# bcgsc/goldrush

Measured on AMD Instinct MI355X. Metric: reads/s through GoldRush-Path (hash + miBF query), higher is better.
Workload: dtype u64

## Files before the change

### goldrush_amd/csrc/grp_device.h

```cpp
#pragma once
#include <hip/hip_runtime.h>
#include <stdint.h>

#define GRP_DEV_MAX_H 16
#define GRP_DEV_MAX_W 32
#define GRP_BUCKET_IDS 13u
#define GRP_NEAR_CW 8u
#define GRP_UNIT_U4 8u
#define GRP_UNIT_DW 32u
#define GRP_UNIT_QW 16u
#define GRP_SUPER_SHIFT 22
#define GRP_CHUNK_BUCKETS 4096u

struct DevSeeds
{
  uint32_t h;
  uint32_t k;
  uint32_t wmax;
  uint32_t n_left;
  uint32_t wide;
  uint32_t weight[GRP_DEV_MAX_H];
  uint32_t span[GRP_DEV_MAX_H];
  uint32_t shift[GRP_DEV_MAX_H][GRP_DEV_MAX_W];
  ulonglong2 tab[GRP_DEV_MAX_H][GRP_DEV_MAX_W][4];
};

struct DevFilter
{
  uint32_t* bv;
  uint4* buckets;
  const uint64_t* super;
  ulonglong2* far;
  uint64_t far_mask;
  unsigned long long* ovf_keys;
  uint32_t* ovf_ids;
  uint64_t ovf_mask;
  uint64_t m;
  uint64_t m_inv;
  uint64_t w_magic;
  uint64_t n_buckets;
  uint64_t pop;
  uint32_t W;
  uint32_t pad;
};

constexpr unsigned long long GRP_CNT_MASK = (1ull << 28) - 1ull;
constexpr uint32_t GRP_EPOCH_MAX = (1u << 10) - 1u;

__host__ __device__ inline uint32_t
grp_cnt(unsigned long long w)
{
  return (uint32_t)(w & GRP_CNT_MASK);
}

__host__ __device__ inline unsigned long long
grp_cnt_with(unsigned long long w, uint32_t count)
{
#if defined(__HIP_DEVICE_COMPILE__)
// ... 163 lines not shown
```

### goldrush_amd/csrc/grp_kernels.inc

```

__device__ inline uint64_t
window_lo(const uint32_t* sBases, uint32_t b)
{
  uint32_t bit = b * 2u;
  uint32_t wi = bit >> 5;
  uint32_t sh = bit & 31u;
  uint64_t lo = (uint64_t)sBases[wi] | ((uint64_t)sBases[wi + 1] << 32);
  uint64_t w = lo >> sh;
  if (sh) {
    w |= (uint64_t)sBases[wi + 2] << (64u - sh);
  }
  return w;
}

struct Win
{
  uint64_t lo;
  const uint32_t* src;
  uint32_t b;
};

__device__ inline Win
window_at(const uint32_t* sBases, uint32_t b)
{
// ... 532 lines not shown
    slot = (slot + 1u) & mask;
  }
}

__device__ inline void
hist_add16(uint32_t* keys, uint32_t* cnt_words, uint32_t cap, uint32_t id, uint32_t* sDistinct, uint32_t limit, uint32_t* sOverflow)
{
  if (*reinterpret_cast<volatile uint32_t*>(sDistinct) >= limit) {
    *sOverflow = 1u;
    return;
  }
  uint32_t slot = __umulhi(id * 2654435761u, cap);
  for (;;) {
    uint32_t old = atomicCAS(&keys[slot], 0u, id);
    if (old == 0u) {
      atomicAdd(sDistinct, 1u);
    }
    if (old == 0u || old == id) {
      atomicAdd(&cnt_words[slot >> 1], 1u << ((slot & 1u) << 4));
      return;
    }
    slot = (slot + 1u == cap) ? 0u : slot + 1u;
  }
}

__device__ inline bool
better(uint32_t c, uint32_t id, uint32_t bc, uint32_t bid)
{
  return (c > bc) || (c == bc && c != 0u && id < bid);
}

template<int WT, bool LEFT, bool RIGHT>
__device__ inline void
seed_halves(const ulonglong2* sTab, const DevSeeds* __restrict__ sd, uint32_t n_left, const Win& win, uint64_t& L, uint64_t& RL, uint64_t& R, uint64_t& RR)
{
  const uint64_t w = win.lo;
  L = RL = R = RR = 0;
  const uint32_t wt = WT > 0 ? (uint32_t)WT : sd->weight[0];
  if (n_left == 8u && wt == 16u) {
    if constexpr (LEFT) {
#pragma unroll
      for (uint32_t i = 0; i < 8u; ++i) {
        const ulonglong2 e = sTab[i * 4u + ((uint32_t)(w >> sd->shift[0][i]) & 3u)];
        L ^= e.x;
        RL ^= e.y;
      }
    }
    if constexpr (RIGHT) {
#pragma unroll
      for (uint32_t i = 8u; i < 16u; ++i) {
        const ulonglong2 e = sTab[i * 4u + ((uint32_t)(w >> sd->shift[0][i]) & 3u)];
        R ^= e.x;
        RR ^= e.y;
      }
    }
    return;
  }
  if constexpr (LEFT) {
    for (uint32_t i = 0; i < n_left; ++i) {
      const ulonglong2 e = sTab[i * 4u + ((uint32_t)(w >> sd->shift[0][i]) & 3u)];
      L ^= e.x;
      RL ^= e.y;
    }
  }
  if constexpr (RIGHT) {
    for (uint32_t i = n_left; i < wt; ++i) {
      const ulonglong2 e = sTab[i * 4u + ((uint32_t)(w >> sd->shift[0][i]) & 3u)];
      R ^= e.x;
      RR ^= e.y;
    }
  }
}

__device__ inline uint64_t
srol_small(uint64_t x, uint32_t n)
{
  const uint64_t M33 = 0x1FFFFFFFFULL, M31 = 0x7FFFFFFFULL;
  const uint64_t lo = x & M33, hi = x >> 33;
  return ((((hi << n) | (hi >> (31u - n))) & M31) << 33) | (((lo << n) | (lo >> (33u - n))) & M33);
}

#define GRP_TILE_FLAGGED 0xFFFFFFFFu

__device__ inline void
store_coherent(unsigned long long* p, unsigned long long v)
{
  __hip_atomic_store(p, v, __ATOMIC_RELAXED, __HIP_MEMORY_SCOPE_AGENT);
}

__device__ inline unsigned long long
load_coherent(const unsigned long long* p)
{
  return __hip_atomic_load(p, __ATOMIC_RELAXED, __HIP_MEMORY_SCOPE_AGENT);
}

__device__ inline uint32_t
ldc(const uint32_t* p)
{
  return __hip_atomic_load(p, __ATOMIC_RELAXED, __HIP_MEMORY_SCOPE_AGENT);
}

__device__ inline void
// ... 1316 lines not shown
  return best_old;
}

template<int H, int FR, int WT, bool ST, bool VER = false, bool GT = false>
__global__ void __launch_bounds__(THREADS, (ST && H <= 3) ? 3 : ((!ST && H >= 4 && H <= 5) ? 3 : 1))
k_query(DevFilter f,
        DevReads rd,
        const DevSeeds* __restrict__ sd,
        uint32_t tile_len,
        uint64_t tile_begin,
        const uint32_t* __restrict__ tile_idx,
        uint32_t hist_cap,
        uint32_t distinct_limit,
        grp_tile_summary* __restrict__ tiles_out,
        grp_id_count* __restrict__ lists_out,
        uint64_t lists_cap,
        unsigned long long* __restrict__ ctr,
        uint32_t* __restrict__ flagged_out,
        uint32_t flagged_cap,
        uint32_t direct_stride,
        uint32_t blk0,
        DevStreamCtl sc,
        DevBatchView bv,
        uint32_t* __restrict__ gtab = nullptr)
{
  if constexpr (VER && !ST) {
    if (bv.redo_count != nullptr && blockIdx.x >= *bv.redo_count) {
      return;
    }
  }
  extern __shared__ uint4 smem4[];
  ulonglong2* sTab = reinterpret_cast<ulonglong2*>(smem4);
  const uint32_t hn = frame_seeds<H>(sd);
  uint32_t* sKeys;
  uint32_t* sCnts;
  uint32_t* sBases;
  if constexpr (GT) {
    sKeys = gtab + (size_t)blockIdx.x * (hist_cap + hist_cap / 2u);
    sCnts = sKeys + hist_cap;
    sBases = reinterpret_cast<uint32_t*>(sTab + hn * sd->wmax * 4u);
  } else {
    sKeys = reinterpret_cast<uint32_t*>(sTab + hn * sd->wmax * 4u);
    sCnts = sKeys + hist_cap;
    sBases = sCnts + hist_cap / 2u;
  }
  auto tab_word = [&](const uint32_t* p) -> uint32_t {
    if constexpr (GT) {
      return __hip_atomic_load(p, __ATOMIC_RELAXED, __HIP_MEMORY_SCOPE_AGENT);
    } else {
      return *p;
    }
  };
  __shared__ uint32_t sListN, sDistinct, sOverflow, sListOff, sListW;
  __shared__ uint32_t sRed[2 * (THREADS / 64)];
  __shared__ uint32_t sBest[2 * (THREADS / 64)];
  __shared__ uint32_t sTile;
  __shared__ unsigned long long sDirectWord;
  __shared__ uint32_t sInsWave[THREADS / 64 + 1];
  __shared__ uint32_t sEv, sAct;
  __shared__ uint32_t sHeldTile[2], sHeldPasses[2];
  __shared__ uint32_t sBuf;
  __shared__ uint32_t sCut;
  __shared__ uint32_t sOwnRedo[2], sOwnRedoN;
  __shared__ uint32_t sWalkEnd;
  __shared__ uint32_t sGen;

  load_tab(sTab, sd);
  constexpr uint32_t STREAM_STOP = 0x40000000u;
  uint32_t nxt = 0;
  uint32_t stop = 0;
  uint32_t my_ev = 0;
  uint32_t phase = 0;
  bool host_abort_seen = false;
  uint32_t ev_next = 0;
  uint32_t pending_event = 0;
  uint32_t* const sFp = (ST && sc.ctl && sc.n_fp) ? reinterpret_cast<uint32_t*>(reinterpret_cast<char*>(smem4) + sc.fp_off) : nullptr;
  if constexpr (ST) {
    if (threadIdx.x == 0) {
      sHeldTile[0] = sHeldTile[1] = STREAM_REDO_NONE;
      sHeldPasses[0] = sHeldPasses[1] = 0u;
      sBuf = 0u;
      sCut = 0u;
      sOwnRedoN = 0u;
      sWalkEnd = 0u;
      sGen = 1u;
      if (sc.dbg) {
        stc(&sc.dbg[blockIdx.x], 0x00000001u);
        stc(&sc.dbg[4095], gridDim.x);
        stc(&sc.dbg[4096 + (blockIdx.x & 1023u)], (uint32_t)wall_clock64());
        stc(&sc.dbg[5120 + (blockIdx.x & 1023u)], (__builtin_amdgcn_s_getreg((16 - 1) << 11 | 4) & 0xFFFFu) | (__builtin_amdgcn_s_getreg((4 - 1) << 11 | 20) << 16));
      }
      if (__hip_atomic_load(sc.abort_host, __ATOMIC_RELAXED, __HIP_MEMORY_SCOPE_SYSTEM)) {
        atomicMin(sc.park, 0u);
        atomicMax(sc.next_tile, STREAM_STOP);
        __hip_atomic_store(sc.abort, 1u, __ATOMIC_RELAXED, __HIP_MEMORY_SCOPE_AGENT);
        stop = 1u;
        host_abort_seen = true;
      }
      if (sc.ctl) {
        uint32_t ph0 = 0;
// ... 220 lines not shown

  uint32_t n_hit = 0, n_miss = 0;
  uint32_t last[H];
#pragma unroll
  for (int s = 0; s < H; ++s) {
    last[s] = Lp - sd->span[s];
  }
  const uint32_t sub = threadIdx.x & 3u;
  const uint32_t quad_base = (threadIdx.x & 63u) & ~3u;

  const uint32_t n_left = (H >= 2 && H <= GRP_H_GROUP && WT != GRP_WT_LONG) ? sd->n_left : 0u;
  constexpr uint32_t OV = (uint32_t)H - 1u, USE = 64u - OV;
  static_assert(THREADS == 256, "the helper-lane layout below is written for four waves per workgroup (my_wave == 3 is the last one, FBH = 3 * USE + 64)");
  constexpr uint32_t FBH = 3u * USE + 64u;
  const uint32_t ftile = frames_per_tile(sd, tile_len);
  const bool helper = n_left != 0u && (ftile + FBH * FR - 1u) / (FBH * FR) == (ftile + THREADS * FR - 1u) / (THREADS * FR);
  const uint32_t FB = helper ? FBH : (uint32_t)THREADS;
  const uint32_t my_wave = threadIdx.x >> 6, my_lane = threadIdx.x & 63u;
  const uint32_t my_off = helper ? (my_wave * USE + my_lane) : threadIdx.x;
  const bool my_real = helper ? (my_wave == 3u || my_lane < USE) : true;
  const bool my_tail_wave = helper ? my_wave == 3u : true;
  const uint32_t passes = (frames + FB * FR - 1u) / (FB * FR);
  uint64_t bk[FR][H];
  uint32_t off[FR][H];
  bool live_j[FR];
  auto positions = [&](uint32_t pp, uint64_t (&bk_)[FR][H], uint32_t (&off_)[FR][H], bool (&lv)[FR]) {
  if (n_left != 0u) {
#pragma unroll
    for (int j = 0; j < FR; ++j) {
      const uint32_t fr_raw = (pp * FR + j) * FB + my_off;
      const uint32_t fr = min(fr_raw, frames - 1u);
      lv[j] = my_real && fr_raw < frames;
      uint64_t hL, hRL, hR, hRR;
      seed_halves<WT, true, true>(sTab, sd, n_left, window_at(sBases, boff + fr), hL, hRL, hR, hRR);
      const uint64_t hv0 = (hL ^ hR) + (hRL ^ hRR);
#pragma unroll
      for (int s = 0; s < H; ++s) {
        uint64_t hv = hv0;
        if (s != 0) {
          uint64_t nR = __shfl_down((unsigned long long)hR, (unsigned)s, 64);
          uint64_t nRR = __shfl_down((unsigned long long)hRR, (unsigned)s, 64);
          if (my_tail_wave && my_lane + (uint32_t)s >= 64u) {
            uint64_t a, b;
            seed_halves<WT, false, true>(sTab, sd, n_left, window_at(sBases, boff + min(fr_raw + (uint32_t)s, frames - 1u)), a, b, nR, nRR);
          }
          if (lv[j]) {
            if (fr <= last[s]) {
              hv = (srol_small(hL, (uint32_t)s) ^ nR) + (hRL ^ srol_small(nRR, (uint32_t)s));
            } else {
              hv = seed_hash_t<WT>(sTab, sd, s, window_at(sBases, boff + last[s]));
            }
          }
        }
        const Probe p = grp_locate(f, hv);
        bk_[j][s] = p.b;
        off_[j][s] = p.off;
        if constexpr (ST) {
          if (fp_cur != nullptr) {
            fp_cur[((pp * FR + (uint32_t)j) * (uint32_t)THREADS + threadIdx.x) * (uint32_t)H + (uint32_t)s] = lv[j] ? slot_fp(p.b, p.off) : 0u;
          }
        }
      }
    }
  } else {
#pragma unroll
    for (int j = 0; j < FR; ++j) {
      const uint32_t fr_raw = (pp * FR + j) * THREADS + threadIdx.x;
      const uint32_t fr = min(fr_raw, frames - 1u);
      lv[j] = fr_raw < frames;
#pragma unroll
      for (int s = 0; s < H; ++s) {
        if (!seed_on<H>(s, frame_seeds<H>(sd))) {
          bk_[j][s] = 0;
          off_[j][s] = 0;
          if constexpr (ST) {
            if (fp_cur != nullptr) {
              fp_cur[((pp * FR + (uint32_t)j) * (uint32_t)THREADS + threadIdx.x) * (uint32_t)H + (uint32_t)s] = 0u;
            }
// ... 794 lines not shown
```

### goldrush_amd/csrc/grpath_hip.hip

```cpp
#include "grp_device.h"
#include "host/gr_tiles_core.hpp"

#include "../../include/grpath.h"

#include <algorithm>
#include <cstdarg>
#include <cstdio>
#include <cstring>
#include <functional>
#include <chrono>
#include <cmath>
#include <mutex>
#include <string>
#include <thread>
#include <vector>


namespace {

thread_local std::string g_create_error;

struct EventPair
{
  hipEvent_t a, b;
  int kind;
};

}


struct QuerySlot
{
  grp_tile_summary* d_tiles = nullptr;
  uint64_t d_tiles_cap = 0;
// ... 375 lines not shown
      c->kstat[ep.kind].ms += (double)ms;
    }
    c->free_events.push_back(ep);
  }
  c->pending.swap(keep);
}

uint64_t
next_pow2_64(uint64_t v)
{
  uint64_t p = 1;
  while (p < v) {
    p <<= 1;
  }
  return p;
}

uint32_t
next_pow2(uint64_t v)
{
  uint32_t p = 1;
  while (p < v) {
    p <<= 1;
  }
  return p;
}

size_t
tab_bytes(const grp_ctx* c)
{
  return (size_t)c->h_seeds.h * c->h_seeds.wmax * 4u * sizeof(ulonglong2);
}

constexpr size_t
bases_bytes(uint32_t nbases)
{
  size_t words = (nbases + 15u) / 16u + 1u + 4u;
  return ((words * 4u + 15u) / 16u) * 16u;
}

inline bool
long_span(const grp_ctx* c)
{
  return c->h_seeds.wide > 1u;
}

inline uint32_t
span0(const grp_ctx* c)
{
  return c->h_seeds.span[0];
}

inline uint32_t
tile_frames(const grp_ctx* c)
{
  return c->params.tile + c->params.k - span0(c);
}

inline uint32_t
tile_parts(const grp_ctx* c)
{
  return (tile_frames(c) + THREADS - 1) / THREADS;
}

template<typename K>
int
// ... 56 lines not shown
  sl.h_qctr = nullptr;
  sl.dec_cap = 0;
  HIP_TRY(c, hipMalloc(&sl.d_dec_raw, (cap + 2) * sizeof(grp_read_decision)));
  HIP_TRY(c, hipHostMalloc(&sl.h_dec_raw, (cap + 2) * sizeof(grp_read_decision), hipHostMallocDefault));
  memset(sl.h_dec_raw, 0, 2 * sizeof(grp_read_decision));
  sl.d_dec = sl.d_dec_raw + 2;
  sl.h_dec = sl.h_dec_raw + 2;
  sl.h_qctr = reinterpret_cast<uint64_t*>(sl.h_dec_raw);
  sl.dec_cap = cap;
  return GRP_OK;
}

template<typename T>
int ensure_dev(grp_ctx* c, T*& p, uint64_t& cap, uint64_t want);

constexpr size_t LDS_PER_WORKGROUP = 160 * 1024 - 512;
static_assert(GRP_DEV_MAX_H * GRP_DEV_MAX_W * 4u * sizeof(ulonglong2) + bases_bytes(GRP_MAX_TILE + GRP_MAX_SPAN + GRP_DEV_MAX_H) <= LDS_PER_WORKGROUP,
              "a tile of the longest span does not fit the LDS beside the seed tables");
constexpr uint32_t GT_SLICE = 256;

struct QueryGeom
{
  uint32_t hist_cap;
  uint32_t distinct_limit;
  size_t lds;
  bool global_table = false;
};

QueryGeom
query_geom(const grp_ctx* c, bool full)
{
  const uint32_t h = c->params.h, tile = c->params.tile;
  const uint64_t max_ids = (uint64_t)tile_frames(c) * h;
  auto lds_of = [&](uint32_t cap) { return tab_bytes(c) + (size_t)cap * 6 + bases_bytes(tile + c->params.k + h); };
  const uint32_t cap_full = (uint32_t)((max_ids + (uint64_t)THREADS * h + 2 + 1023) / 1024 * 1024);
  const uint32_t forced_small = c->env_small_hist;
  QueryGeom g;
  g.hist_cap = cap_full;
  if (!full) {
    if (forced_small && forced_small < cap_full && forced_small > (uint32_t)THREADS * h + 64) {
      g.hist_cap = forced_small;
    } else if (lds_of(cap_full) > 52 * 1024) {
      const size_t fixed = lds_of(0);
      const uint32_t cap = (uint32_t)((52 * 1024 - std::min<size_t>(fixed, 40 * 1024)) / 6 / 1024 * 1024);
      if (cap > (uint32_t)THREADS * h + 1024 && cap < cap_full) {
        g.hist_cap = cap;
      }
    }
    if (g.hist_cap == cap_full && lds_of(cap_full) > LDS_PER_WORKGROUP) {
      const size_t fixed = lds_of(0);
      const uint32_t cap = fixed < LDS_PER_WORKGROUP ? (uint32_t)((LDS_PER_WORKGROUP - fixed) / 6 / 1024 * 1024) : 0u;
      if (cap > (uint32_t)THREADS * h + 64) {
        g.hist_cap = cap;
      }
    }
  }
  g.distinct_limit = g.hist_cap - THREADS * h - 1;
  g.lds = lds_of(g.hist_cap);
  if (full && g.lds > LDS_PER_WORKGROUP) {
    g.global_table = true;
    g.lds = lds_of(0);
  }
  return g;
}

template<int HH, int QWT>
int
launch_query_wt(grp_ctx* c, const grp_reads* r, uint64_t n_launch, uint64_t t0, const uint32_t* d_tile_idx, const QueryGeom& g, uint64_t list_cap, grp_tile_summary* out_tiles, grp_id_count* out_lists, uint32_t direct_stride, const DevStreamCtl* stream_ctl,
                uint32_t blk0, bool list_flags, bool plain)
{
  if (!out_tiles) {
    out_tiles = c->q->d_tiles;
    out_lists = c->q->d_lists;
  }
  size_t launch_lds = g.lds;
  auto go = [&](auto kern) -> int {
    int rc = ensure_lds(c, kern, launch_lds);
    if (rc != GRP_OK) {
      return rc;
    }
    if (stream_ctl && stream_ctl->ctl) {
      {
        DevFilter a_f = c->f;
        DevReads a_rd = r->dev;
        const DevSeeds* a_sd = c->d_seeds;
        uint32_t a_tile = c->params.tile;
        uint64_t a_t0 = t0;
        const uint32_t* a_idx = d_tile_idx;
        uint32_t a_cap = g.hist_cap, a_lim = g.distinct_limit;
        grp_tile_summary* a_tiles = out_tiles;
        grp_id_count* a_lists = out_lists;
        uint64_t a_lcap = list_cap;
        unsigned long long* a_ctr = reinterpret_cast<unsigned long long*>(c->q->d_qctr);
        uint32_t* a_flag = (d_tile_idx && !list_flags) ? nullptr : c->q->d_flag_idx;
        uint32_t a_fcap = (uint32_t)c->q->d_flag_cap, a_ds = direct_stride, a_blk0 = blk0;
        DevStreamCtl a_sc = *stream_ctl;
// ... 147 lines not shown
    }
    sd.weight[s] = w;
    sd.wmax = std::max(sd.wmax, w);
  }
  if (sd.wmax == 0) {
    return set_err(c, GRP_ERR_INVALID, "seeds have weight 0");
  }
  c->uniform_weight = sd.wmax;
  for (uint32_t s2 = 0; s2 < sd.h; ++s2) {
    if (sd.weight[s2] != sd.wmax) {
      c->uniform_weight = 0;
    }
  }
  const uint32_t span = sd.span[sd.h - 1];
  sd.wide = (span > 64) ? 2u : (span > 32) ? 1u : 0u;
  if (sd.wide) {
    c->uniform_weight = 0;
  }
  sd.n_left = 0;
  {
    const char* e = getenv("GRP_SHARED_HALVES");
    const std::string& s0 = c->seeds[0];
    const size_t cut = s0.size() / 2;
    bool family = sd.h >= 2 && !(e && !strcmp(e, "off"));
    for (uint32_t s2 = 1; s2 < sd.h && family; ++s2) {
      family = c->seeds[s2] == s0.substr(0, cut) + std::string(s2, '0') + s0.substr(cut);
    }
    uint32_t nl = 0;
    for (size_t q = 0; q < cut; ++q) {
      nl += s0[q] == '1';
    }
    if (family && nl > 0 && nl < sd.weight[0] && !sd.wide) {
      sd.n_left = nl;
    }
  }
  return GRP_OK;
}

}

extern "C" {

const char*
grp_last_error(const grp_ctx* ctx)
{
  return ctx ? ctx->err.c_str() : g_create_error.c_str();
}

int
grp_create(const grp_params* p, grp_ctx** out)
{
  if (!p || !out || p->struct_size != sizeof(grp_params)) {
    return set_err(nullptr, GRP_ERR_INVALID, "grp_create: bad params / struct_size");
  }
  *out = nullptr;
  if (p->h < 1 || p->h > GRP_MAX_SEEDS) {
    return set_err(nullptr, GRP_ERR_INVALID, "h=%u: this implementation supports 1 to %d spaced seeds", p->h, GRP_MAX_SEEDS);
  }
  if (p->k < 1 || p->k > GRP_MAX_SPAN || p->k + p->h - 1 > GRP_MAX_SPAN) {
    return set_err(nullptr, GRP_ERR_INVALID, "k=%u h=%u: the longest seed spans k+h-1=%u bases, this implementation supports spans of 1 to %d bases", p->k, p->h, p->k + p->h - 1, GRP_MAX_SPAN);
  }
  if (p->tile < p->k + p->h - 1) {
    return set_err(nullptr, GRP_ERR_INVALID, "tile length %u shorter than the longest seed span %u", p->tile, p->k + p->h - 1);
  }
  if (p->tile > GRP_MAX_TILE) {
    return set_err(nullptr, GRP_ERR_INVALID, "tile length %u: a tile holds at most 65 535 frames (an ID's count per tile is 16 bits)", p->tile);
// ... 2453 lines not shown
```

### goldrush_amd/csrc/host/gr_capi.cpp

```cpp
#include "../../../include/grpath_host.h"
#include "gr_classifier.hpp"
#include "gr_params.hpp"
#include "gr_opts.hpp"
#include <algorithm>
#include <sstream>
#include "gr_tiles.hpp"
#include "gr_fastq.hpp"

#include <cstddef>
#include <cstring>
#include <new>

extern "C" {

int
gr_make_seed_pattern(const char* preset, unsigned k, unsigned weight, unsigned h, char* out, size_t stride, int log_to_stderr)
{
  if (!out || k / 2 == 0) {
    return -1;
  }
  auto seeds = gr::make_seed_pattern(preset ? preset : "", k, weight, h, log_to_stderr != 0);
  for (unsigned i = 0; i < h; ++i) {
    if (seeds[i].size() + 1 > stride) {
      return -1;
    }
    std::memcpy(out + (size_t)i * stride, seeds[i].c_str(), seeds[i].size() + 1);
  }
  return 0;
}

uint64_t
gr_hash_universe(uint64_t weight, uint64_t genome_size, uint64_t hash_num)
{
  return gr::hash_universe(weight, genome_size, hash_num);
}

uint64_t
gr_calc_optimal_size(uint64_t entries, unsigned hash_num, double occupancy)
{
  return gr::calc_optimal_size(entries, hash_num, occupancy);
}

void
gr_calc_phred_average(const char* qual, size_t n, uint32_t* avg, uint32_t* delta)
{
  gr::calc_phred_average(qual, n, *avg, *delta);
}

double
gr_sum_phred(const char* qual, size_t n)
{
  return gr::sum_phred(qual, n);
}

int
gr_process_options_dump(int argc, char** argv, char* out, size_t cap)
{
  gr::Opts o;
  const int rc = gr::process_options(o, argc, argv);
  std::ostringstream ss;
  ss << "assigned_max=" << o.assigned_max << "\n"
// ... 228 lines not shown
```

### goldrush_amd/host.py

```python
from __future__ import annotations

import ctypes as C
import os

import numpy as np

from . import native

LIB_PATH = os.path.join(native.LIB_DIR, "libgrpath_host.so")
CLI_PATH = os.path.join(os.path.dirname(native.LIB_DIR), "bin", "goldrush-path")

_vp = C.c_void_p
decision_dtype = np.dtype([("kind", "<u4"), ("num_tiles", "<u4"), ("num_assigned", "<u4"), ("trim_start", "<u4"), ("trim_end", "<u4"),
                           ("hits", "<u4"), ("misses", "<u4"), ("pad", "<u4")])
KIND_NAMES = {2: "insert_whole", 3: "assigned_all", 4: "insert_trimmed", 5: "assigned"}


class gr_read_decision(C.Structure):
    _fields_ = [(n, C.c_uint32) for n in ("kind", "num_tiles", "num_assigned", "trim_start", "trim_end", "hits", "misses", "pad")]


class gr_commit(C.Structure):
    _fields_ = [("read", C.c_uint32), ("dec", gr_read_decision), ("first_id", C.c_uint32), ("path", C.c_uint64)]

# ... 45 lines not shown
    ("fastq_records", C.CFUNCTYPE(C.c_int, _vp, _vp)),
    ("fastq_pack", C.CFUNCTYPE(C.c_int, _vp, _vp, _vp, C.c_uint32, C.POINTER(_vp))),
    ("fastq_free", C.CFUNCTYPE(None, _vp)),
    ("stream_begin_resumable", C.CFUNCTYPE(C.c_int, _vp, _vp, C.c_uint32, C.c_uint32, _vp, C.c_uint32, _vp)),
    ("stream_insert", C.CFUNCTYPE(C.c_int, _vp, C.c_uint32, C.c_uint32, C.c_uint32, C.c_uint32, C.c_uint32, C.c_uint32, C.c_uint32, C.POINTER(C.c_uint32))),
    ("comm_unique_id", C.CFUNCTYPE(C.c_int, _vp, C.c_size_t)),
    ("comm_init", C.CFUNCTYPE(C.c_int, _vp, _vp, C.c_uint32, C.c_uint32)),
    ("bv_merge_ranks", C.CFUNCTYPE(C.c_int, _vp)),
    ("bv_words", C.CFUNCTYPE(C.c_int, _vp, C.POINTER(C.c_uint64))),
    ("bv_export_words", C.CFUNCTYPE(C.c_int, _vp, C.c_uint64, C.c_uint64, _vp)),
    ("bv_or_words", C.CFUNCTYPE(C.c_int, _vp, C.c_uint64, C.c_uint64, _vp)),
    ("fastq_pin", C.CFUNCTYPE(C.c_int, _vp, _vp, C.c_uint64)),
    ("fastq_unpin", C.CFUNCTYPE(C.c_int, _vp)),
    ("batch_verify", C.CFUNCTYPE(C.c_int, _vp, _vp, C.c_uint32, C.c_uint32, C.c_uint32, _vp, _vp, _vp)),
    ("window_overlap", C.CFUNCTYPE(C.c_int, _vp, _vp, C.c_uint32, C.c_uint32, C.c_uint32, _vp)),
    ("stream_begin_striped_resumable", C.CFUNCTYPE(C.c_int, _vp, _vp, C.c_uint32, C.c_uint32, _vp, C.c_uint32, C.c_uint32, C.c_uint32, C.c_uint32, _vp)),
    ("stream_resumable", C.CFUNCTYPE(C.c_int, _vp, C.c_uint32)),
    ("stream_insert_done", C.CFUNCTYPE(C.c_int, _vp, C.c_uint32)),
    ("fastq_prefetch", C.CFUNCTYPE(C.c_int, _vp, _vp, C.c_uint64)),
    ("occupancy_hint", C.CFUNCTYPE(C.c_int, _vp, C.c_double)),
]


class grp_engine_vt(C.Structure):
    _fields_ = VT_TYPES


COMMIT_FN = C.CFUNCTYPE(C.c_double, _vp, C.POINTER(gr_commit))
ROLLOVER_FN = C.CFUNCTYPE(None, _vp, C.c_uint64)
ALLGATHER_FN = C.CFUNCTYPE(C.c_int, _vp, _vp, C.c_uint64, _vp)

SIGNATURES = {
    "gr_make_seed_pattern": (C.c_int, [C.c_char_p, C.c_uint, C.c_uint, C.c_uint, _vp, C.c_size_t, C.c_int]),
    "gr_hash_universe": (C.c_uint64, [C.c_uint64, C.c_uint64, C.c_uint64]),
    "gr_calc_optimal_size": (C.c_uint64, [C.c_uint64, C.c_uint, C.c_double]),
    "gr_calc_phred_average": (None, [C.c_char_p, C.c_size_t, C.POINTER(C.c_uint32), C.POINTER(C.c_uint32)]),
    "gr_sum_phred": (C.c_double, [C.c_char_p, C.c_size_t]),
    "gr_pack_2bit": (C.c_int, [C.c_char_p, C.c_size_t, _vp]),
    "gr_effective_cpus": (C.c_uint, []),
    "gr_process_options_dump": (C.c_int, [C.c_int, C.POINTER(C.c_char_p), C.c_char_p, C.c_size_t]),
    "gr_ntcard_sbits": (C.c_uint, [C.c_uint64]),
    "gr_ntcard_f0": (C.c_uint64, [C.c_uint64, C.c_uint64, C.c_uint]),
    "gr_ntcard_split": (C.c_size_t, [C.c_char_p, C.c_size_t, C.c_uint, C.c_uint, _vp, _vp, _vp, C.c_size_t]),
    "gr_decide_read": (None, [C.c_size_t, C.c_size_t, C.c_size_t, C.c_size_t, _vp, _vp, C.POINTER(gr_read_decision)]),
    "gr_smooth_tiles": (C.c_size_t, [C.c_size_t, _vp, _vp, C.c_size_t, _vp, _vp]),
    "gr_find_longest_stretch": (None, [_vp, C.c_size_t, C.POINTER(C.c_long), C.POINTER(C.c_long)]),
    "gr_eval_flanks": (C.c_int, [C.c_long, C.c_long, _vp, C.c_size_t, C.POINTER(C.c_size_t), C.POINTER(C.c_size_t)]),
    "gr_classifier_create": (C.c_int, [C.POINTER(gr_classifier_params), C.POINTER(grp_engine_vt), _vp, C.POINTER(_vp)]),
    "gr_classifier_destroy": (None, [_vp]),
    "gr_classifier_set_allgather": (None, [_vp, _vp, _vp]),
    "gr_classifier_set_debug": (None, [_vp, _vp]),
    "gr_classifier_keep_commits": (None, [_vp, C.c_uint32, C.c_uint32, C.c_uint32, C.c_uint32]),
    "gr_classifier_kept_commits": (C.c_size_t, [_vp, _vp, C.c_size_t]),
    "gr_shm_allgather_open": (_vp, [C.c_uint32, C.c_uint32, C.c_char_p, C.c_double]),
    "gr_shm_allgather": (C.c_int, [_vp, _vp, C.c_uint64, _vp]),
    "gr_fill_merge_plan": (C.c_int, [C.POINTER(grp_engine_vt), _vp, _vp, C.c_uint32, C.c_uint32, C.c_int]),
    "gr_fill_merge_run": (C.c_int, [C.POINTER(grp_engine_vt), _vp, _vp, C.c_uint32, C.c_uint32, C.c_int]),
    "gr_ranks_same_u64": (C.c_int, [_vp, C.c_uint32, C.c_uint64]),
    "gr_ranks_share_device": (C.c_int, [_vp, C.c_uint32, C.c_int]),
    "gr_shm_allgather_close": (None, [_vp]),
    "gr_classifier_set_callbacks": (None, [_vp, COMMIT_FN, ROLLOVER_FN, ALLGATHER_FN, _vp]),
    "gr_classifier_run": (C.c_int, [_vp, _vp, _vp, C.c_uint32, _vp, C.c_uint32, C.POINTER(C.c_int)]),
    "gr_classifier_run_range": (C.c_int, [_vp, _vp, _vp, C.c_uint32, C.c_uint32, _vp, C.c_uint32, C.POINTER(C.c_int)]),
    "gr_classifier_error": (C.c_char_p, [_vp]),
    "gr_classifier_get_state": (None, [_vp, C.POINTER(gr_classifier_state)]),
    "gr_path_main": (C.c_int, [C.c_int, C.POINTER(C.c_char_p), C.POINTER(grp_engine_vt)]),
# ... 188 lines not shown
```

### include/grpath_host.h

```cpp
#ifndef GRPATH_HOST_H
#define GRPATH_HOST_H

#include "grpath.h"
#include "grpath_ingest.h"

#ifdef __cplusplus
extern "C" {
#endif

typedef struct
{
  int (*create)(const grp_params*, void** ctx_out);
  void (*destroy)(void* ctx);
  const char* (*last_error)(const void* ctx);
  int (*reads_upload)(void* ctx, const uint32_t* packed, const uint64_t* word_off, const uint32_t* len, uint32_t n_reads, void** out);
  void (*reads_free)(void* reads);
  int (*bv_insert)(void* ctx, const void* reads, uint32_t first, uint32_t count);
  int (*finalize)(void* ctx, uint64_t* pop);
  int (*query_tiles)(void* ctx, const void* reads, uint32_t first, uint32_t count, grp_tile_summary* tiles, grp_id_count* lists, uint64_t list_cap, uint64_t* list_used, grp_query_stats* stats);
  int (*insert_tiles)(void* ctx, const void* reads, uint32_t read_idx, uint32_t tile_start, uint32_t tile_end, uint32_t id);
  int (*reset_ids)(void* ctx);
  int (*sync)(void* ctx);
  int (*classify_reads)(void* ctx, const void* reads, uint32_t first, uint32_t count, const grp_decide_params* params, grp_read_decision* out);
  int (*insert_read)(void* ctx, const void* reads, uint32_t read_idx, uint32_t tile_start, uint32_t tile_end, uint32_t block_tiles, uint32_t first_id, uint32_t id_offset);
// ... 5 lines not shown
  int (*stream_end)(void* ctx, uint32_t slot, uint32_t* reads_decided);
  int (*batch_insert)(void* ctx, const void* reads, const grp_batch_insert* inserts, uint32_t n_inserts, uint32_t block_tiles, uint32_t first_read);
  int (*batch_classify)(void* ctx, const void* reads, uint32_t first, uint32_t count, const grp_decide_params* params, const uint32_t* id_floor, grp_read_decision* out);
  int (*batch_undo)(void* ctx, uint32_t from_read, uint32_t id_floor);
  int (*batch_end)(void* ctx);
  int (*ntcard_begin)(void* ctx, uint32_t sbits);
  int (*ntcard_add)(void* ctx, const void* reads, uint32_t first, uint32_t count, const uint32_t* stale_extra);
  int (*ntcard_finish)(void* ctx, uint64_t* zero_buckets);
  int (*set_filter_size)(void* ctx, uint64_t m);
  int (*fastq_parse)(void* ctx, const char* text, uint64_t n_bytes, int final_chunk, void** fq_out, uint64_t* n_records, uint64_t* bytes_consumed, int* stopped);
  int (*fastq_records)(void* fq, grp_fastq_record* out);
  int (*fastq_pack)(void* ctx, void* fq, const uint32_t* sel, uint32_t n_sel, void** reads_out);
  void (*fastq_free)(void* fq);
  int (*stream_begin_resumable)(void* ctx, const void* reads, uint32_t first, uint32_t count, const grp_decide_params* params, uint32_t slot, const grp_read_decision** decisions);
  int (*stream_insert)(void* ctx, uint32_t slot, uint32_t read_idx, uint32_t tile_start, uint32_t tile_end, uint32_t block_tiles, uint32_t first_id, uint32_t id_offset, uint32_t* generation);
  int (*comm_unique_id)(void* out, size_t cap);
  int (*comm_init)(void* ctx, const void* unique_id, uint32_t world, uint32_t rank);
  int (*bv_merge_ranks)(void* ctx);
  int (*bv_words)(const void* ctx, uint64_t* n_words32);
  int (*bv_export_words)(void* ctx, uint64_t first, uint64_t n_words32, uint32_t* words);
  int (*bv_or_words)(void* ctx, uint64_t first, uint64_t n_words32, const uint32_t* words);
  int (*fastq_pin)(void* ctx, const char* buffer, uint64_t n_bytes);
  int (*fastq_unpin)(void* ctx);
  int (*batch_verify)(void* ctx, const void* reads, uint32_t first, uint32_t count, uint32_t extra, const grp_decide_params* params, const uint32_t* id_floor, grp_read_decision* out);
  int (*window_overlap)(void* ctx, const void* reads, uint32_t first, uint32_t count, uint32_t threshold, uint32_t* prev_out);
  int (*stream_begin_striped_resumable)(void* ctx, const void* reads, uint32_t first, uint32_t count, const grp_decide_params* params, uint32_t slot, uint32_t stripe_reads, uint32_t n_owners, uint32_t owner, const grp_read_decision** decisions);
  int (*stream_resumable)(void* ctx, uint32_t slot);
  int (*stream_insert_done)(void* ctx, uint32_t slot);
  int (*fastq_prefetch)(void* ctx, const char* text, uint64_t n_bytes);
  int (*occupancy_hint)(void* ctx, double occupancy);
} grp_engine_vt;

int gr_make_seed_pattern(const char* preset, unsigned k, unsigned weight, unsigned h, char* out, size_t stride, int log_to_stderr);
uint64_t gr_hash_universe(uint64_t weight, uint64_t genome_size, uint64_t hash_num);
uint64_t gr_calc_optimal_size(uint64_t entries, unsigned hash_num, double occupancy);
void gr_calc_phred_average(const char* qual, size_t n, uint32_t* avg, uint32_t* delta);
double gr_sum_phred(const char* qual, size_t n);
int gr_pack_2bit(const char* seq, size_t n, uint32_t* out_words);
unsigned gr_ntcard_sbits(uint64_t input_bytes);
uint64_t gr_ntcard_f0(uint64_t zero0, uint64_t zero1, unsigned sbits);
size_t gr_ntcard_split(const char* seq, size_t n, unsigned k, unsigned h, uint64_t* run_off, uint64_t* run_len, uint32_t* extra, size_t cap);
int gr_process_options_dump(int argc, char** argv, char* out, size_t cap);
unsigned gr_effective_cpus(void);

typedef grp_read_decision gr_read_decision;

void gr_decide_read(size_t threshold, size_t unassigned_min, size_t assigned_max, size_t num_tiles, const grp_tile_summary* tiles, const grp_id_count* lists, gr_read_decision* out);
size_t gr_smooth_tiles(size_t num_tiles, const grp_tile_summary* tiles, const grp_id_count* lists, size_t threshold, uint32_t* ids_out, uint8_t* bools_out);
void gr_find_longest_stretch(const uint8_t* bools, size_t num_tiles, long* start, long* end);
int gr_eval_flanks(long longest_start, long longest_end, const uint32_t* ids, size_t num_tiles, size_t* trim_start, size_t* trim_end);

typedef struct
{
  uint32_t struct_size;
  uint32_t tile_length;
  uint32_t block_size;
  uint32_t threshold;
  uint32_t unassigned_min;
  uint32_t assigned_max;
  uint32_t kmer_size;
  uint32_t hash_num;
  uint64_t target_bases;
  uint64_t max_paths;
  int32_t silver_path;
  int32_t verbose;
  uint32_t max_window;
// ... 71 lines not shown
```

Measured before the change: 477,100.

## Merge adjacent spaced-seed positions into combined lookup tables and precompute wrap tails

Adds a host-side seed plan that groups runs of adjacent care positions into pair tables (16 entries each), stored in LDS after the per-position tables. This roughly halves the number of LDS lookups and XORs per seed hash. The plan's LDS budget is derived from occupancy shares. The tail wave now computes its wrapped right-half hash once, before the shuffle loop, and uses a single __shfl per shift instead of recomputing inside the loop. The cost is extra LDS, which could hurt occupancy, plus more host-side planning logic.

```diff
diff --git a/goldrush_amd/csrc/grp_device.h b/goldrush_amd/csrc/grp_device.h
--- a/goldrush_amd/csrc/grp_device.h
+++ b/goldrush_amd/csrc/grp_device.h
@@ -4,6 +4,7 @@
 
 #define GRP_DEV_MAX_H 16
 #define GRP_DEV_MAX_W 32
+#define GRP_PLAN_MAX_ENTRIES 512
 #define GRP_BUCKET_IDS 13u
 #define GRP_NEAR_CW 8u
 #define GRP_UNIT_U4 8u
@@ -23,7 +24,14 @@
   uint32_t span[GRP_DEV_MAX_H];
   uint32_t shift[GRP_DEV_MAX_H][GRP_DEV_MAX_W];
   ulonglong2 tab[GRP_DEV_MAX_H][GRP_DEV_MAX_W][4];
-};
+  uint32_t g_nl, g_n, g_rshift, g_extra, g_shape;
+  uint32_t g_shift[GRP_DEV_MAX_W], g_bits[GRP_DEV_MAX_W], g_off[GRP_DEV_MAX_W];
+  ulonglong2 g_tab[GRP_PLAN_MAX_ENTRIES];
+};
+
+#define GRP_SHAPE_GENERIC 0u
+#define GRP_SHAPE_PAIRS16 1u
+#define GRP_SHAPE_SINGLES16 2u
 
 struct DevFilter
 {
diff --git a/goldrush_amd/csrc/grp_kernels.inc b/goldrush_amd/csrc/grp_kernels.inc
--- a/goldrush_amd/csrc/grp_kernels.inc
+++ b/goldrush_amd/csrc/grp_kernels.inc
@@ -588,42 +588,59 @@
 
 template<int WT, bool LEFT, bool RIGHT>
 __device__ inline void
-seed_halves(const ulonglong2* sTab, const DevSeeds* __restrict__ sd, uint32_t n_left, const Win& win, uint64_t& L, uint64_t& RL, uint64_t& R, uint64_t& RR)
-{
-  const uint64_t w = win.lo;
+seed_halves(const ulonglong2* sTab, const DevSeeds* __restrict__ sd, const Win& win, uint64_t& L, uint64_t& RL, uint64_t& R, uint64_t& RR)
+{
   L = RL = R = RR = 0;
-  const uint32_t wt = WT > 0 ? (uint32_t)WT : sd->weight[0];
-  if (n_left == 8u && wt == 16u) {
+  const uint32_t wl = (uint32_t)win.lo;
+  const uint32_t wr = (uint32_t)(win.lo >> sd->g_rshift);
+  auto look = [&](uint32_t word, uint32_t g, uint32_t bits, uint32_t at, uint64_t& f, uint64_t& r) {
+    const ulonglong2 e = sTab[at + __builtin_amdgcn_ubfe(word, sd->g_shift[g], bits)];
+    f ^= e.x;
+    r ^= e.y;
+  };
+  const uint32_t shape = sd->g_shape;
+  if (shape == GRP_SHAPE_PAIRS16) {
+    const uint32_t pairs = sd->g_off[1];
     if constexpr (LEFT) {
+      look(wl, 0u, 2u, 0u, L, RL);
+      look(wl, 1u, 4u, pairs, L, RL);
+      look(wl, 2u, 4u, pairs + 16u, L, RL);
+      look(wl, 3u, 4u, pairs + 32u, L, RL);
+      look(wl, 4u, 2u, 7u * 4u, L, RL);
+    }
+    if constexpr (RIGHT) {
+      look(wr, 5u, 2u, 8u * 4u, R, RR);
+      look(wr, 6u, 4u, pairs + 48u, R, RR);
+      look(wr, 7u, 4u, pairs + 64u, R, RR);
+      look(wr, 8u, 4u, pairs + 80u, R, RR);
+      look(wr, 9u, 2u, 15u * 4u, R, RR);
+    }
+    return;
+  }
+  if (shape == GRP_SHAPE_SINGLES16) {
+    if constexpr (LEFT) {
 #pragma unroll
       for (uint32_t i = 0; i < 8u; ++i) {
-        const ulonglong2 e = sTab[i * 4u + ((uint32_t)(w >> sd->shift[0][i]) & 3u)];
-        L ^= e.x;
-        RL ^= e.y;
+        look(wl, i, 2u, i * 4u, L, RL);
       }
     }
     if constexpr (RIGHT) {
 #pragma unroll
       for (uint32_t i = 8u; i < 16u; ++i) {
-        const ulonglong2 e = sTab[i * 4u + ((uint32_t)(w >> sd->shift[0][i]) & 3u)];
-        R ^= e.x;
-        RR ^= e.y;
+        look(wr, i, 2u, i * 4u, R, RR);
       }
     }
     return;
   }
+  const uint32_t gl = sd->g_nl, gn = sd->g_n;
   if constexpr (LEFT) {
-    for (uint32_t i = 0; i < n_left; ++i) {
-      const ulonglong2 e = sTab[i * 4u + ((uint32_t)(w >> sd->shift[0][i]) & 3u)];
-      L ^= e.x;
-      RL ^= e.y;
+    for (uint32_t g = 0; g < gl; ++g) {
+      look(wl, g, sd->g_bits[g], sd->g_off[g], L, RL);
     }
   }
   if constexpr (RIGHT) {
-    for (uint32_t i = n_left; i < wt; ++i) {
-      const ulonglong2 e = sTab[i * 4u + ((uint32_t)(w >> sd->shift[0][i]) & 3u)];
-      R ^= e.x;
-      RR ^= e.y;
+    for (uint32_t g = gl; g < gn; ++g) {
+      look(wr, g, sd->g_bits[g], sd->g_off[g], R, RR);
     }
   }
 }
@@ -2006,15 +2023,16 @@
   extern __shared__ uint4 smem4[];
   ulonglong2* sTab = reinterpret_cast<ulonglong2*>(smem4);
   const uint32_t hn = frame_seeds<H>(sd);
+  const uint32_t n_tab = hn * sd->wmax * 4u + sd->g_extra;
   uint32_t* sKeys;
   uint32_t* sCnts;
   uint32_t* sBases;
   if constexpr (GT) {
     sKeys = gtab + (size_t)blockIdx.x * (hist_cap + hist_cap / 2u);
     sCnts = sKeys + hist_cap;
-    sBases = reinterpret_cast<uint32_t*>(sTab + hn * sd->wmax * 4u);
+    sBases = reinterpret_cast<uint32_t*>(sTab + n_tab);
   } else {
-    sKeys = reinterpret_cast<uint32_t*>(sTab + hn * sd->wmax * 4u);
+    sKeys = reinterpret_cast<uint32_t*>(sTab + n_tab);
     sCnts = sKeys + hist_cap;
     sBases = sCnts + hist_cap / 2u;
   }
@@ -2040,6 +2058,9 @@
   __shared__ uint32_t sGen;
 
   load_tab(sTab, sd);
+  for (uint32_t i = threadIdx.x; i < sd->g_extra; i += blockDim.x) {
+    sTab[hn * sd->wmax * 4u + i] = sd->g_tab[i];
+  }
   constexpr uint32_t STREAM_STOP = 0x40000000u;
   uint32_t nxt = 0;
   uint32_t stop = 0;
@@ -2326,18 +2347,20 @@
       const uint32_t fr = min(fr_raw, frames - 1u);
       lv[j] = my_real && fr_raw < frames;
       uint64_t hL, hRL, hR, hRR;
-      seed_halves<WT, true, true>(sTab, sd, n_left, window_at(sBases, boff + fr), hL, hRL, hR, hRR);
+      seed_halves<WT, true, true>(sTab, sd, window_at(sBases, boff + fr), hL, hRL, hR, hRR);
       const uint64_t hv0 = (hL ^ hR) + (hRL ^ hRR);
+      uint64_t tR = 0, tRR = 0;
+      if (my_tail_wave && my_lane < OV) {
+        uint64_t a, b;
+        seed_halves<WT, false, true>(sTab, sd, window_at(sBases, boff + min(fr_raw + 64u, frames - 1u)), a, b, tR, tRR);
+      }
 #pragma unroll
       for (int s = 0; s < H; ++s) {
         uint64_t hv = hv0;
         if (s != 0) {
-          uint64_t nR = __shfl_down((unsigned long long)hR, (unsigned)s, 64);
-          uint64_t nRR = __shfl_down((unsigned long long)hRR, (unsigned)s, 64);
-          if (my_tail_wave && my_lane + (uint32_t)s >= 64u) {
-            uint64_t a, b;
-            seed_halves<WT, false, true>(sTab, sd, n_left, window_at(sBases, boff + min(fr_raw + (uint32_t)s, frames - 1u)), a, b, nR, nRR);
-          }
+          const bool wrapped = my_tail_wave && my_lane < (uint32_t)s;
+          const uint64_t nR = __shfl((unsigned long long)(wrapped ? tR : hR), (int)((my_lane + (uint32_t)s) & 63u), 64);
+          const uint64_t nRR = __shfl((unsigned long long)(wrapped ? tRR : hRR), (int)((my_lane + (uint32_t)s) & 63u), 64);
           if (lv[j]) {
             if (fr <= last[s]) {
               hv = (srol_small(hL, (uint32_t)s) ^ nR) + (hRL ^ srol_small(nRR, (uint32_t)s));
diff --git a/goldrush_amd/csrc/grpath_hip.hip b/goldrush_amd/csrc/grpath_hip.hip
--- a/goldrush_amd/csrc/grpath_hip.hip
+++ b/goldrush_amd/csrc/grpath_hip.hip
@@ -1,5 +1,6 @@
 #include "grp_device.h"
 #include "host/gr_tiles_core.hpp"
+#include "host/gr_seed_plan.hpp"
 
 #include "../../include/grpath.h"
 
@@ -441,6 +442,12 @@
   return (size_t)c->h_seeds.h * c->h_seeds.wmax * 4u * sizeof(ulonglong2);
 }
 
+size_t
+plan_bytes(const grp_ctx* c)
+{
+  return (size_t)c->h_seeds.g_extra * sizeof(ulonglong2);
+}
+
 constexpr size_t
 bases_bytes(uint32_t nbases)
 {
@@ -563,7 +570,7 @@
 {
   const uint32_t h = c->params.h, tile = c->params.tile;
   const uint64_t max_ids = (uint64_t)tile_frames(c) * h;
-  auto lds_of = [&](uint32_t cap) { return tab_bytes(c) + (size_t)cap * 6 + bases_bytes(tile + c->params.k + h); };
+  auto lds_of = [&](uint32_t cap) { return tab_bytes(c) + plan_bytes(c) + (size_t)cap * 6 + bases_bytes(tile + c->params.k + h); };
   const uint32_t cap_full = (uint32_t)((max_ids + (uint64_t)THREADS * h + 2 + 1023) / 1024 * 1024);
   const uint32_t forced_small = c->env_small_hist;
   QueryGeom g;
@@ -593,6 +600,43 @@
     g.lds = lds_of(0);
   }
   return g;
+}
+
+constexpr size_t LDS_ALLOC_UNIT = 1280, LDS_SHARE_3WG_UNITS = 42, QUERY_STATIC_LDS = 512;
+constexpr size_t LDS_SHARE_3WG = LDS_SHARE_3WG_UNITS * LDS_ALLOC_UNIT - QUERY_STATIC_LDS;
+static_assert(3 * LDS_SHARE_3WG_UNITS * LDS_ALLOC_UNIT <= 160 * 1024, "three shares exceed a CU's LDS");
+
+uint32_t
+stream_fp_words(const grp_ctx* c)
+{
+  const uint32_t h = c->params.h;
+  const uint32_t fb = 3u * (64u - (h - 1u)) + 64u;
+  const uint32_t passes = (tile_frames(c) + fb - 1u) / fb;
+  return passes * (uint32_t)THREADS * h;
+}
+
+uint32_t
+plan_budget_entries(const grp_ctx* c)
+{
+  const size_t base = query_geom(c, false).lds;
+  const size_t fp = (size_t)stream_fp_words(c) * 4u;
+  size_t limit = LDS_PER_WORKGROUP, held = base;
+  if (base <= LDS_SHARE_3WG) {
+    limit = LDS_SHARE_3WG;
+    for (int nf = 2; nf >= 1; --nf) {
+      if (base + (size_t)nf * fp <= LDS_SHARE_3WG) {
+        held = base + (size_t)nf * fp;
+        break;
+      }
+    }
+  } else if (base <= LDS_PER_WORKGROUP / 2) {
+    limit = LDS_PER_WORKGROUP / 2 / LDS_ALLOC_UNIT * LDS_ALLOC_UNIT;
+  }
+  size_t room = limit > held ? limit - held : 0;
+  if (base <= 52 * 1024) {
+    room = std::min<size_t>(room, 52 * 1024 - base);
+  }
+  return (uint32_t)std::min<size_t>(room / sizeof(ulonglong2), GRP_PLAN_MAX_ENTRIES);
 }
 
 template<int HH, int QWT>
@@ -806,6 +850,44 @@
     }
     if (family && nl > 0 && nl < sd.weight[0] && !sd.wide) {
       sd.n_left = nl;
+    }
+  }
+  if (sd.n_left != 0 && sd.h <= (uint32_t)GRP_H_GROUP) {
+    const char* e = getenv("GRP_HALF_GROUP");
+    const uint32_t max_width = e ? (uint32_t)std::max(1, std::min((int)gr::SEED_PLAN_MAX_WIDTH, atoi(e))) : 2u;
+    const uint32_t cap0 = query_geom(c, false).hist_cap;
+    const char* eb = getenv("GRP_PLAN_ENTRIES");
+    const uint32_t budget = eb ? (uint32_t)std::max(0, std::min((int)GRP_PLAN_MAX_ENTRIES, atoi(eb))) : plan_budget_entries(c);
+    for (int attempt = 0; attempt < 2; ++attempt) {
+      const gr::SeedPlan p = gr::make_seed_plan(c->seeds[0], attempt ? 1u : max_width, attempt ? 0u : budget);
+      if (p.groups.empty() || p.groups.size() > GRP_DEV_MAX_W || p.n_extra > GRP_PLAN_MAX_ENTRIES) {
+        return set_err(c, GRP_ERR_INVALID, "no look-up plan for seed 0 (%zu groups, %u entries)", p.groups.size(), p.n_extra);
+      }
+      sd.g_nl = p.n_left_groups;
+      sd.g_n = (uint32_t)p.groups.size();
+      sd.g_rshift = p.rshift;
+      sd.g_extra = p.n_extra;
+      bool pairs16 = sd.n_left == 8 && sd.weight[0] == 16 && sd.g_nl == 5 && sd.g_n == 10, singles16 = sd.n_left == 8 && sd.weight[0] == 16 && sd.g_n == 16;
+      static const uint32_t first16[10] = { 0, 1, 3, 5, 7, 8, 9, 11, 13, 15 }, width16[10] = { 1, 2, 2, 2, 1, 1, 2, 2, 2, 1 };
+      uint32_t pair_off = 0;
+      for (uint32_t g = 0; g < sd.g_n; ++g) {
+        const gr::SeedGroup& gp = p.groups[g];
+        sd.g_shift[g] = gp.shift;
+        sd.g_bits[g] = 2u * gp.width;
+        sd.g_off[g] = gp.width == 1 ? gp.first * 4u : sd.h * sd.wmax * 4u + gp.off;
+        pairs16 = pairs16 && g < 10 && gp.first == first16[g] && gp.width == width16[g] && (gp.width == 1 || gp.off == pair_off);
+        pair_off += gp.width == 2 ? 16u : 0u;
+        singles16 = singles16 && gp.width == 1 && gp.first == g;
+      }
+      sd.g_shape = pairs16 ? GRP_SHAPE_PAIRS16 : singles16 ? GRP_SHAPE_SINGLES16 : GRP_SHAPE_GENERIC;
+      static_assert(sizeof(ulonglong2) == 2 * sizeof(uint64_t), "table entries are {fwd, rev}");
+      gr::fill_seed_plan(p, reinterpret_cast<const uint64_t*>(&sd.tab[0][0][0]), reinterpret_cast<uint64_t*>(&sd.g_tab[0]));
+      if (attempt == 0 && !e && !eb && sd.n_left == 8 && sd.weight[0] == 16 && sd.g_shape == GRP_SHAPE_GENERIC) {
+        continue;
+      }
+      if (query_geom(c, false).hist_cap == cap0 && query_geom(c, true).lds <= LDS_PER_WORKGROUP) {
+        break;
+      }
     }
   }
   return GRP_OK;
diff --git a/goldrush_amd/csrc/host/gr_capi.cpp b/goldrush_amd/csrc/host/gr_capi.cpp
--- a/goldrush_amd/csrc/host/gr_capi.cpp
+++ b/goldrush_amd/csrc/host/gr_capi.cpp
@@ -2,6 +2,7 @@
 #include "gr_classifier.hpp"
 #include "gr_params.hpp"
 #include "gr_opts.hpp"
+#include "gr_seed_plan.hpp"
 #include <algorithm>
 #include <sstream>
 #include "gr_tiles.hpp"
@@ -27,6 +28,32 @@
     std::memcpy(out + (size_t)i * stride, seeds[i].c_str(), seeds[i].size() + 1);
   }
   return 0;
+}
+
+int
+gr_seed_plan(const char* seed0, unsigned max_width, unsigned budget_entries, const uint64_t* tab, uint32_t* groups, size_t groups_cap, uint32_t* head, uint64_t* extra, size_t extra_cap)
+{
+  if (!seed0 || !groups || !head) {
+    return -1;
+  }
+  const gr::SeedPlan p = gr::make_seed_plan(seed0, max_width, budget_entries);
+  if (p.groups.size() > groups_cap || (extra && p.n_extra > extra_cap)) {
+    return -1;
+  }
+  head[0] = p.n_left_groups;
+  head[1] = p.rshift;
+  head[2] = p.n_extra;
+  for (size_t i = 0; i < p.groups.size(); ++i) {
+    const gr::SeedGroup& g = p.groups[i];
+    groups[i * 4 + 0] = g.first;
+    groups[i * 4 + 1] = g.width;
+    groups[i * 4 + 2] = g.shift;
+    groups[i * 4 + 3] = g.off;
+  }
+  if (tab && extra) {
+    gr::fill_seed_plan(p, tab, extra);
+  }
+  return (int)p.groups.size();
 }
 
 uint64_t
diff --git a/goldrush_amd/csrc/host/gr_seed_plan.hpp b/goldrush_amd/csrc/host/gr_seed_plan.hpp
--- /dev/null
+++ b/goldrush_amd/csrc/host/gr_seed_plan.hpp
@@ -0,0 +1,96 @@
+#pragma once
+#include <cstdint>
+#include <string>
+#include <vector>
+
+namespace gr {
+
+constexpr uint32_t SEED_PLAN_MAX_WIDTH = 4;
+
+struct SeedGroup
+{
+  uint32_t first;
+  uint32_t width;
+  uint32_t shift;
+  uint32_t off;
+};
+
+struct SeedPlan
+{
+  uint32_t n_left_groups = 0;
+  uint32_t rshift = 0;
+  uint32_t n_extra = 0;
+  std::vector<SeedGroup> groups;
+};
+
+inline SeedPlan
+make_seed_plan(const std::string& seed0, uint32_t max_width, uint32_t budget_entries)
+{
+  SeedPlan p;
+  const size_t n = seed0.size(), cut = n / 2;
+  if (n == 0 || cut > 16 || n - cut > 16) {
+    return p;
+  }
+  max_width = max_width < 1 ? 1 : (max_width > SEED_PLAN_MAX_WIDTH ? SEED_PLAN_MAX_WIDTH : max_width);
+  p.rshift = 2u * (uint32_t)cut;
+  uint32_t care = 0;
+  for (int half = 0; half < 2; ++half) {
+    const size_t lo = half ? cut : 0, hi = half ? n : cut;
+    size_t q = lo;
+    while (q < hi) {
+      if (seed0[q] != '1') {
+        ++q;
+        continue;
+      }
+      size_t run = 1;
+      while (q + run < hi && seed0[q + run] == '1') {
+        ++run;
+      }
+      for (size_t at = 0; at < run;) {
+        uint32_t w = (uint32_t)((run - at < max_width) ? run - at : max_width);
+        while (w > 1 && (1u << (2u * w)) > budget_entries - p.n_extra) {
+          --w;
+        }
+        SeedGroup g;
+        g.first = care;
+        g.width = w;
+        g.shift = 2u * (uint32_t)(q + at - lo);
+        g.off = 0;
+        if (w > 1) {
+          g.off = p.n_extra;
+          p.n_extra += 1u << (2u * w);
+        }
+        p.groups.push_back(g);
+        care += w;
+        at += w;
+      }
+      q += run;
+    }
+    if (half == 0) {
+      p.n_left_groups = (uint32_t)p.groups.size();
+    }
+  }
+  return p;
+}
+
+inline void
+fill_seed_plan(const SeedPlan& p, const uint64_t* tab, uint64_t* out)
+{
+  for (const SeedGroup& g : p.groups) {
+    if (g.width < 2) {
+      continue;
+    }
+    for (uint32_t idx = 0; idx < (1u << (2u * g.width)); ++idx) {
+      uint64_t f = 0, r = 0;
+      for (uint32_t j = 0; j < g.width; ++j) {
+        const uint64_t* e = tab + ((size_t)(g.first + j) * 4u + ((idx >> (2u * j)) & 3u)) * 2u;
+        f ^= e[0];
+        r ^= e[1];
+      }
+      out[(size_t)(g.off + idx) * 2u] = f;
+      out[(size_t)(g.off + idx) * 2u + 1u] = r;
+    }
+  }
+}
+
+}
diff --git a/goldrush_amd/host.py b/goldrush_amd/host.py
--- a/goldrush_amd/host.py
+++ b/goldrush_amd/host.py
@@ -101,6 +101,7 @@
 
 SIGNATURES = {
     "gr_make_seed_pattern": (C.c_int, [C.c_char_p, C.c_uint, C.c_uint, C.c_uint, _vp, C.c_size_t, C.c_int]),
+    "gr_seed_plan": (C.c_int, [C.c_char_p, C.c_uint, C.c_uint, _vp, _vp, C.c_size_t, _vp, _vp, C.c_size_t]),
     "gr_hash_universe": (C.c_uint64, [C.c_uint64, C.c_uint64, C.c_uint64]),
     "gr_calc_optimal_size": (C.c_uint64, [C.c_uint64, C.c_uint, C.c_double]),
     "gr_calc_phred_average": (None, [C.c_char_p, C.c_size_t, C.POINTER(C.c_uint32), C.POINTER(C.c_uint32)]),
diff --git a/include/grpath_host.h b/include/grpath_host.h
--- a/include/grpath_host.h
+++ b/include/grpath_host.h
@@ -61,6 +61,7 @@
 } grp_engine_vt;
 
 int gr_make_seed_pattern(const char* preset, unsigned k, unsigned weight, unsigned h, char* out, size_t stride, int log_to_stderr);
+int gr_seed_plan(const char* seed0, unsigned max_width, unsigned budget_entries, const uint64_t* tab, uint32_t* groups, size_t groups_cap, uint32_t* head, uint64_t* extra, size_t extra_cap);
 uint64_t gr_hash_universe(uint64_t weight, uint64_t genome_size, uint64_t hash_num);
 uint64_t gr_calc_optimal_size(uint64_t entries, unsigned hash_num, double occupancy);
 void gr_calc_phred_average(const char* qual, size_t n, uint32_t* avg, uint32_t* delta);
```

New measurement: 482,500 (median of 6 runs). Within noise of the previous version (+1.1%).
